# shivangchopra11/MedMoE

Measured on AMD Instinct MI355X. Metric: image-text pairs/sec at global batch 1024, higher is better.
Workload: dtype bf16; 1 GPU; cfg2: ViT-B/16 + 12-layer text tower (frozen), 8 experts top-2, 224x224x3 + 77 tokens, fwd+bwd+clip+Adam; global_batch=1024, per_gpu_batch=1024, parallelism=dp1

## Files before the change

medmoe_amd/csrc/embed.hip:

```cpp
#include "common.h"

template <typename InT>
__global__ __launch_bounds__(256) void patchify_kernel(const InT* __restrict__ img, bf16_t* __restrict__ out, int B,
                                                       int C, int H, int W, int p, int ld) {
  const int gw = W / p, gh = H / p;
  const long long total = (long long)B * C * H * gw;
  for (long long i = blockIdx.x * 256LL + threadIdx.x; i < total; i += (long long)gridDim.x * 256) {
    const int gx = i % gw;
    long long r = i / gw;
    const int y = r % H; r /= H;
    const int c = r % C;
    const int b = r / C;
    const int gy = y / p, py = y - gy * p;
    const InT* src = img + (((long long)b * C + c) * H + y) * W + gx * p;
    bf16_t* dst = out + ((long long)b * gh * gw + gy * gw + gx) * ld + c * p * p + py * p;
    for (int k = 0; k < p; ++k) {
      if constexpr (sizeof(InT) == 4) dst[k] = f2bf(src[k]); else dst[k] = src[k];
    }
  }
}

extern "C" int medmoe_patchify_ld(const void* img, void* out, int B, int C, int H, int W, int patch, int in_f32, int ld,
                                  hipStream_t stream) {
  if (!img || !out) return MM_ERR_ARG;
  if (B <= 0 || C <= 0 || patch <= 0 || (H % patch) || (W % patch) || ld < C * patch * patch || (ld % 8)) return MM_ERR_SHAPE;
  const long long total = (long long)B * C * H * (W / patch);
  const int grid = (int)min((total + 255) / 256, (long long)256 * 16);
  if (in_f32)
    hipLaunchKernelGGL(patchify_kernel<float>, dim3(grid), dim3(256), 0, stream, (const float*)img, (bf16_t*)out, B, C, H, W, patch, ld);
  else
    hipLaunchKernelGGL(patchify_kernel<bf16_t>, dim3(grid), dim3(256), 0, stream, (const bf16_t*)img, (bf16_t*)out, B, C, H, W, patch, ld);
  return mm_check_launch();
}

extern "C" int medmoe_patchify(const void* img, void* out, int B, int C, int H, int W, int patch, int in_f32,
                               hipStream_t stream) {
  if ((C * patch * patch) % 8) return MM_ERR_SHAPE;
  return medmoe_patchify_ld(img, out, B, C, H, W, patch, in_f32, C * patch * patch, stream);
}

__global__ __launch_bounds__(256) void init_tokens_kernel(bf16_t* __restrict__ x, const float* __restrict__ cls,
                                                          const float* __restrict__ pos, int B, int Nt, int D) {
  const long long total = (long long)B * Nt * D / 4;
  for (long long i = blockIdx.x * 256LL + threadIdx.x; i < total; i += (long long)gridDim.x * 256) {
    const long long e = i * 4;
    const int col = e % D;
    const int t = (e / D) % Nt;
    float4 v = *(const float4*)(pos + (long long)t * D + col);
    if (t == 0) {
      const float4 c = *(const float4*)(cls + col);
      v.x += c.x; v.y += c.y; v.z += c.z; v.w += c.w;
    }
    uint2 o; o.x = pack2bf(v.x, v.y); o.y = pack2bf(v.z, v.w);
    *(uint2*)(x + e) = o;
  }
}

extern "C" int medmoe_init_tokens(void* x, const float* cls, const float* pos, int B, int Nt, int D,
                                  hipStream_t stream) {
  if (!x || !cls || !pos) return MM_ERR_ARG;
  if (B <= 0 || Nt <= 0 || D <= 0 || (D % 4)) return MM_ERR_SHAPE;
  const long long total = (long long)B * Nt * D / 4;
  const int grid = (int)min((total + 255) / 256, (long long)256 * 16);
  hipLaunchKernelGGL(init_tokens_kernel, dim3(grid), dim3(256), 0, stream, (bf16_t*)x, cls, pos, B, Nt, D);
  return mm_check_launch();
}

__global__ __launch_bounds__(256) void pos_cls_grad_kernel(const bf16_t* __restrict__ dx, float* __restrict__ dpos,
                                                           float* __restrict__ dcls, int B, int Nt, int D) {
  const int t = blockIdx.x, col = (blockIdx.y * 256 + threadIdx.x) * 2;
  if (col >= D) return;
  const bf16_t* src = dx + (long long)t * D + col;
  const long long bs = (long long)Nt * D;
  float s0 = 0.f, s1 = 0.f;
  int b = 0;
  for (; b + 8 <= B; b += 8) {
    uint32_t v[8];
#pragma unroll
    for (int u = 0; u < 8; ++u) v[u] = *(const uint32_t*)(src + (b + u) * bs);
#pragma unroll
    for (int u = 0; u < 8; ++u) { s0 += __uint_as_float(v[u] << 16); s1 += __uint_as_float(v[u] & 0xffff0000u); }
  }
  for (; b < B; ++b) {
    const uint32_t v = *(const uint32_t*)(src + b * bs);
    s0 += __uint_as_float(v << 16); s1 += __uint_as_float(v & 0xffff0000u);
  }
  dpos[(long long)t * D + col] += s0; dpos[(long long)t * D + col + 1] += s1;
  if (t == 0) { dcls[col] += s0; dcls[col + 1] += s1; }
}

extern "C" int medmoe_pos_cls_grad(const void* dx, float* dpos, float* dcls, int B, int Nt, int D,
                                   hipStream_t stream) {
  if (!dx || !dpos || !dcls) return MM_ERR_ARG;
  if (B <= 0 || Nt <= 0 || D <= 0 || (D % 2)) return MM_ERR_SHAPE;
  hipLaunchKernelGGL(pos_cls_grad_kernel, dim3(Nt, (D + 511) / 512), dim3(256), 0, stream, (const bf16_t*)dx, dpos,
                     dcls, B, Nt, D);
  return mm_check_launch();
}

__global__ __launch_bounds__(256) void text_embed_ln_kernel(const int* __restrict__ ids, const int* __restrict__ tts,
                                                            const float* __restrict__ word, const float* __restrict__ pos,
                                                            const float* __restrict__ type, const float* __restrict__ gamma,
                                                            const float* __restrict__ beta, bf16_t* __restrict__ out,
                                                            int rows, int T, int D, int vocab, float eps, const int* __restrict__ src_of_row,
                                                            const int* __restrict__ rows_dev) {
  const int lane = threadIdx.x & 63, wid = threadIdx.x >> 6;
  const int n4 = D >> 2;
  if (rows_dev) rows = min(rows, *rows_dev);
  for (int row = blockIdx.x * 4 + wid; row < rows; row += gridDim.x * 4) {
    const int src = src_of_row ? src_of_row[row] : row;
    const int t = src % T;
    int id = ids[src]; id = min(max(id, 0), vocab - 1);
    const int tt = tts ? min(max(tts[src], 0), 1) : 0;
    float4 v[8];
    float s = 0.f;
#pragma unroll
    for (int i = 0; i < 8; ++i) {
      const int c = lane + i * 64;
      if (c < n4) {
        const float4 a = *(const float4*)(word + (long long)id * D + c * 4);
        const float4 p = *(const float4*)(pos + (long long)t * D + c * 4);
        const float4 y = *(const float4*)(type + (long long)tt * D + c * 4);
        v[i] = make_float4(a.x + p.x + y.x, a.y + p.y + y.y, a.z + p.z + y.z, a.w + p.w + y.w);
        s += v[i].x + v[i].y + v[i].z + v[i].w;
      }
    }
    const float mean = wave_sum(s) / (float)D;
    float sq = 0.f;
#pragma unroll
    for (int i = 0; i < 8; ++i)
      if (lane + i * 64 < n4) {
        const float a = v[i].x - mean, b = v[i].y - mean, c = v[i].z - mean, d = v[i].w - mean;
        sq += a * a + b * b + c * c + d * d;
      }
    const float rstd = rsqrtf(wave_sum(sq) / (float)D + eps);
#pragma unroll
    for (int i = 0; i < 8; ++i) {
      const int c = lane + i * 64;
      if (c < n4) {
        const float4 g = *(const float4*)(gamma + c * 4), b = *(const float4*)(beta + c * 4);
        uint2 o;
        o.x = pack2bf((v[i].x - mean) * rstd * g.x + b.x, (v[i].y - mean) * rstd * g.y + b.y);
        o.y = pack2bf((v[i].z - mean) * rstd * g.z + b.z, (v[i].w - mean) * rstd * g.w + b.w);
        *(uint2*)(out + (long long)row * D + c * 4) = o;
      }
    }
  }
}

extern "C" int medmoe_text_embed_ln(const int* ids, const int* type_ids, const float* word, const float* pos,
                                    const float* type, const float* gamma, const float* beta, void* out,
                                    int B, int T, int D, int vocab, float eps, hipStream_t stream) {
  if (!ids || !word || !pos || !type || !gamma || !beta || !out) return MM_ERR_ARG;
  if (B <= 0 || T <= 0 || D <= 0 || (D % 4) || D > 2048 || vocab <= 0) return MM_ERR_SHAPE;
  const int rows = B * T;
  const int grid = min((rows + 3) / 4, 256 * 8);
  hipLaunchKernelGGL(text_embed_ln_kernel, dim3(grid), dim3(256), 0, stream, ids, type_ids, word, pos, type, gamma,
                     beta, (bf16_t*)out, rows, T, D, vocab, eps, (const int*)nullptr, (const int*)nullptr);
  return mm_check_launch();
}

__global__ __launch_bounds__(1024) void text_pack_kernel(const unsigned char* __restrict__ mask, int* __restrict__ tok_row,
                                                         int* __restrict__ src_of_row, int* __restrict__ seq_off, int* __restrict__ count,
                                                         int B, int T) {
  __shared__ int sh[1024];
  const int b = threadIdx.x;
  int n = 0;
  if (b < B)
    for (int t = 0; t < T; ++t) n += mask[b * T + t] ? 1 : 0;
  sh[b] = n;
  __syncthreads();
  for (int o = 1; o < 1024; o <<= 1) {
    const int v = (b >= o) ? sh[b - o] : 0;
    __syncthreads();
    sh[b] += v;
    __syncthreads();
  }
  if (b < B) {
    int r = sh[b] - n;
    seq_off[b] = r;
    for (int t = 0; t < T; ++t) {
      if (mask[b * T + t]) { tok_row[b * T + t] = r; src_of_row[r] = b * T + t; ++r; }
      else tok_row[b * T + t] = -1;
    }
    if (b == B - 1) { seq_off[B] = sh[b]; count[0] = sh[b]; }
  }
}

extern "C" int medmoe_text_pack(const unsigned char* mask, int* tok_row, int* src_of_row, int* seq_off, int* count, int B, int T,
                                hipStream_t stream) {
  if (!mask || !tok_row || !src_of_row || !seq_off || !count) return MM_ERR_ARG;
  if (B <= 0 || B > 1024 || T <= 0) return MM_ERR_SHAPE;
  hipLaunchKernelGGL(text_pack_kernel, dim3(1), dim3(1024), 0, stream, mask, tok_row, src_of_row, seq_off, count, B, T);
  return mm_check_launch();
}

__global__ __launch_bounds__(256) void segment_map_kernel(const void* __restrict__ ids_, int ids64, const unsigned char* __restrict__ is_cont,
                                                          const unsigned char* __restrict__ starts_bracket, int* __restrict__ seg,
                                                          int* __restrict__ cap, int B, int T, int vocab, int sep_id) {
  const int b = blockIdx.x * 256 + threadIdx.x;
  if (b >= B) return;
  auto id_at = [&](int t) -> int {
    const long long v = ids64 ? ((const long long*)ids_)[(long long)b * T + t] : (long long)((const int*)ids_)[(long long)b * T + t];
    return (int)min(max(v, 0ll), (long long)vocab - 1);
  };
  int sep_pos = T;
  for (int t = 0; t < T; ++t)
    if (id_at(t) == sep_id) { sep_pos = t; break; }
  int c = -1, at_sep = 0;
  for (int t = 0; t < T; ++t) {
    const int id = id_at(t);
    const bool st = t == 0 || (t <= sep_pos && !is_cont[id]);
    c += st ? 1 : 0;
    seg[(long long)b * T + t] = c;
    if (t == sep_pos) at_sep = c;
  }
  const int n_words = sep_pos < T ? at_sep + 1 : c;
  int prev = -1, n_real = 0;
  for (int t = 0; t < T; ++t) {
    const int w = seg[(long long)b * T + t];
    const bool keep = t <= sep_pos && w < n_words;
    if (keep && w != prev) {
      n_real += starts_bracket[id_at(t)] ? 0 : 1;
      prev = w;
    }
    if (!keep) seg[(long long)b * T + t] = -1;
  }
  cap[b] = n_real + 1;
}

__global__ __launch_bounds__(256) void segment_map_wave_kernel(const void* __restrict__ ids_, int ids64, const unsigned char* __restrict__ is_cont,
                                                               const unsigned char* __restrict__ starts_bracket, int* __restrict__ seg,
                                                               int* __restrict__ cap, int B, int T, int vocab, int sep_id) {
  const int lane = threadIdx.x & 63;
  const int b = blockIdx.x * 4 + (threadIdx.x >> 6);
  if (b >= B) return;
  int id[2], cont[2], brk[2];
#pragma unroll
  for (int u = 0; u < 2; ++u) {
    const int t = 2 * lane + u;
    id[u] = -1; cont[u] = 0; brk[u] = 0;
    if (t < T) {
      const long long v = ids64 ? ((const long long*)ids_)[(long long)b * T + t] : (long long)((const int*)ids_)[(long long)b * T + t];
      id[u] = (int)min(max(v, 0ll), (long long)vocab - 1);
      cont[u] = is_cont[id[u]]; brk[u] = starts_bracket[id[u]];
    }
  }
  int sep_pos = T;
#pragma unroll
  for (int u = 1; u >= 0; --u) if (2 * lane + u < T && id[u] == sep_id) sep_pos = 2 * lane + u;
#pragma unroll
  for (int m = 32; m > 0; m >>= 1) sep_pos = min(sep_pos, __shfl_xor(sep_pos, m, 64));
  int st[2];
#pragma unroll
  for (int u = 0; u < 2; ++u) { const int t = 2 * lane + u; st[u] = (t < T && (t == 0 || (t <= sep_pos && !cont[u]))) ? 1 : 0; }
  int incl = st[0] + st[1];
#pragma unroll
  for (int m = 1; m < 64; m <<= 1) { const int v = __shfl_up(incl, m, 64); if (lane >= m) incl += v; }
  const int base = incl - st[0] - st[1];
  int c[2] = {base + st[0] - 1, base + st[0] + st[1] - 1};
  const int probe = sep_pos < T ? sep_pos : T - 1;
  int at = (probe >> 1) == lane ? c[probe & 1] : 0;
#pragma unroll
  for (int m = 32; m > 0; m >>= 1) at += __shfl_xor(at, m, 64);
  const int n_words = sep_pos < T ? at + 1 : at;
  int n_real = 0;
#pragma unroll
  for (int u = 0; u < 2; ++u) {
// ... 393 lines not shown
```

medmoe_amd/csrc/gemm.hip:

```cpp
#include "common.h"
#include "det_plan.h"
#include <utility>

#define BM 128
#define BN 128
#define BK 64

__device__ __attribute__((aligned(256))) bf16_t g_zero_page[2048];

struct GemmNTArgs {
  const bf16_t* A; const bf16_t* B; void* C;
  const float* bias; const bf16_t* residual; bf16_t* aux;
  const int* a_rowmap; const int* c_rowmap; const int4* tiles; const int* tile_count;
  long long strideB; long long strideBias;
  int M, N, K, lda, ldb, ldc, ldr, ldaux;
  int n_tiles_n, max_tiles_m;
  float alpha; int epi; int out_f32; int col_perm;
  const int* m_dev;
};

static int g_use_nt256 = 1, g_use_nt512 = 1, g_use_tn512 = 1, g_tn_rows = 1024, g_nt_max_grid = 256, g_use_scores512 = 1, g_use_nt4w = 1, g_use_tn4w = 1, g_tn_min_rows = 2048, g_tn_rows4w = 0, g_scores_skip_epi = 0;
#ifdef NT_EXPERIMENT
__device__ int g_nt_dbg_skip = 0;
#define NT_X(...) __VA_ARGS__
#else
#define NT_X(...)
#endif
#ifdef NT_TIMING
__device__ unsigned long long g_nt_timing[8 * 8];
#define NT_T(...) __VA_ARGS__
__device__ __forceinline__ long long nt_clk() {
  __builtin_amdgcn_sched_barrier(0); const long long c = clock64(); __builtin_amdgcn_sched_barrier(0); return c;
}
#else
#define NT_T(...)
#endif
extern int g_attn_resident;
extern int g_sa_rows;
extern int g_attn_rt13;
static int g_last_nt_kernel = -1;
extern "C" int medmoe_last_gemm_nt_kernel() { return g_last_nt_kernel; }
extern int g_ln_one_row;
int g_use_nt_direct = 1;
extern "C" int medmoe_set_option(int key, int value) {
  if (key == 16) { g_ln_one_row = value; return MM_OK; }
  if (key == 17) { g_use_nt_direct = value; return MM_OK; }
  if (key == 1) { g_use_nt256 = value; return MM_OK; }
  if (key == 2) { g_use_nt512 = value; return MM_OK; }
  if (key == 3) { g_use_tn512 = value; return MM_OK; }
  if (key == 4 && value >= 256) { g_tn_rows = value; return MM_OK; }
  if (key == 5 && value >= 1 && value <= 256) { g_nt_max_grid = value; return MM_OK; }
  if (key == 6) { g_use_scores512 = value; return MM_OK; }
  if (key == 7) { g_use_nt4w = value; return MM_OK; }
  if (key == 8) { g_use_tn4w = value; return MM_OK; }
  if (key == 9 && value >= 64) { g_tn_min_rows = value; return MM_OK; }
  if (key == 12) { g_scores_skip_epi = value; return MM_OK; }
  if (key == 15 && (value == 0 || value == 448 || value == 512)) { g_attn_rt13 = value; return MM_OK; }
  if (key == 13 && value >= 0) { g_sa_rows = value; return MM_OK; }
  if (key == 11) { g_attn_resident = value; return MM_OK; }
  if (key == 10 && value >= 0) { g_tn_rows4w = value; return MM_OK; }
  return MM_ERR_ARG;
}

enum { EPI_NONE = 0, EPI_GELU = 1, EPI_RELU = 2, EPI_MUL_DGELU = 3, EPI_MUL_DRELU = 4, EPI_GELU_DAUX = 5, EPI_MUL_AUX = 6 };

struct ParkedTile {
  uint4 c[8];
  int m_base, n_base, n_items, next;
};

typedef unsigned u32x4e_t __attribute__((ext_vector_type(4)));
template <bool PARK, int TM0 = 0, int TMS = 4, int TN0 = 0, int TNS = 4, bool LDSX = false>
__device__ __forceinline__ int nt_epilogue(const GemmNTArgs& p, f32x4_t (&acc)[TMS][TNS], int m_base, int m_end,
                                           int n_base, int group, int frag_row, int frag_q, ParkedTile* park, unsigned lds_x = 0u) {
  int n_stores = 0;
  const int pg = ((frag_q & 1) << 1) | (frag_q >> 1);
  long long mc[4];
  bool mok[4];
#pragma unroll
  for (int tm = 0; tm < 4; ++tm) {
    const int m = m_base + tm * 16 + frag_row;
    mok[tm] = m < m_end;
    const int mr = min(m, m_end - 1);
    mc[tm] = p.c_rowmap ? (long long)p.c_rowmap[mr] : (long long)mr;
  }
  int nn[4];
  bool nok[4];
#pragma unroll
  for (int tn = 0; tn < 4; ++tn) {
    const int n = n_base + tn * 16 + pg * 4;
    nok[tn] = n < p.N;
    nn[tn] = min(n, p.N - 4);
  }
  float4 b4[4];
  if (p.bias) {
    const float* bias = p.bias + (long long)group * p.strideBias;
#pragma unroll
    for (int tn = 0; tn < 4; ++tn) b4[tn] = *(const float4*)(bias + nn[tn]);
  }
  uint2 res[4][4], axv[4][4];
  if (p.residual) {
#pragma unroll
    for (int tm = 0; tm < 4; ++tm)
#pragma unroll
      for (int tn = 0; tn < 4; ++tn) res[tm][tn] = *(const uint2*)(p.residual + mc[tm] * p.ldr + nn[tn]);
  }
  const bool mul_epi = p.epi == EPI_MUL_DGELU || p.epi == EPI_MUL_DRELU || p.epi == EPI_MUL_AUX;
  if (mul_epi) {
#pragma unroll
    for (int tm = 0; tm < 4; ++tm)
#pragma unroll
      for (int tn = 0; tn < 4; ++tn) axv[tm][tn] = *(const uint2*)(p.aux + mc[tm] * p.ldaux + nn[tn]);
  }
  const bool wide = !p.out_f32 && !p.col_perm && (p.N & 7) == 0;
  const bool upper = frag_q >= 2;
  auto store_pair = [&](bf16_t* base, long long ld, int tm, int j, uint2 lo, uint2 hi, bool is_aux) {
    auto r0 = __builtin_amdgcn_permlane32_swap(lo.x, hi.x, false, false);
    auto r1 = __builtin_amdgcn_permlane32_swap(lo.y, hi.y, false, false);
    if constexpr (PARK) {
      if (!is_aux) { park->c[tm * 2 + j] = make_uint4(r0[0], r1[0], r0[1], r1[1]); return; }
    }
    if constexpr (LDSX) {
      const int row_l = (tm & 1) * 16 + frag_row, slot = (2 * j + (upper ? 1 : 0)) * 2 + (frag_q & 1);
      const unsigned a = lds_x + (is_aux ? 4096u : 0u) + row_l * 128 + ((slot ^ ((row_l >> 1) & 7)) << 4);
      const u32x4e_t d = {(unsigned)r0[0], (unsigned)r1[0], (unsigned)r0[1], (unsigned)r1[1]};
      asm volatile("ds_write_b128 %0, %1" :: "v"(a), "v"(d) : "memory");
      return;
    }
// ... 722 lines not shown
    const float f[8] = {lo[i][0], lo[i][1], lo[i][2], lo[i][3], hi[i][0], hi[i][1], hi[i][2], hi[i][3]};
    float o[8], dg[8];
#pragma unroll
    for (int k = 0; k < 4; ++k) {
      if constexpr (GELU) {
        f32x2_t g_, d_;
        gelu_and_grad2((f32x2_t){f[2 * k], f[2 * k + 1]}, g_, d_);
        o[2 * k] = g_[0]; o[2 * k + 1] = g_[1]; dg[2 * k] = d_[0]; dg[2 * k + 1] = d_[1];
      } else {
        const float z0 = __uint_as_float(r[i][k] << 16), z1 = __uint_as_float(r[i][k] & 0xffff0000u);
        o[2 * k] = MUL ? f[2 * k] * z0 : f[2 * k] + z0;
        o[2 * k + 1] = MUL ? f[2 * k + 1] * z1 : f[2 * k + 1] + z1;
      }
    }
    const u32x4e_t pk = {pack2bf(o[0], o[1]), pack2bf(o[2], o[3]), pack2bf(o[4], o[5]), pack2bf(o[6], o[7])};
    __builtin_nontemporal_store(pk, (u32x4e_t*)((bf16_t*)p.C + (long long)(mb + tmh * 16 + i * 8 + rl) * p.ldc + nb + tnq * 16 + c8 * 8));
    if constexpr (GELU) {
      const u32x4e_t pd = {pack2bf(dg[0], dg[1]), pack2bf(dg[2], dg[3]), pack2bf(dg[4], dg[5]), pack2bf(dg[6], dg[7])};
      __builtin_nontemporal_store(pd, (u32x4e_t*)(p.aux + (long long)(mb + tmh * 16 + i * 8 + rl) * p.ldaux + nb + tnq * 16 + c8 * 8));
    }
  }
}
template <int SPEC>
__device__ __forceinline__ int nt4w_epilogue_rows(const GemmNTArgs& p, f32x4_t (&acc)[8][8], int mb, int nb, int frag_row, int frag_q,
                                                  unsigned lx) {
  constexpr bool MUL = (SPEC & 7) == EPI_MUL_AUX;
  asm volatile("" : "+v"(frag_row), "+v"(frag_q));
  const int lane = frag_q * 16 + frag_row, rl = lane >> 3, c8 = lane & 7;
  const int pg = ((frag_q & 1) << 1) | (frag_q >> 1);
  float4 b4[8];
  float zero = 0.f;
  asm volatile("" : "+v"(zero));
#pragma unroll
  for (int tn = 0; tn < 8; ++tn) b4[tn] = (SPEC & 8) ? *(const float4*)(p.bias + nb + tn * 16 + pg * 4) : make_float4(zero, zero, zero, zero);
  u32x4e_t ra[4], rb[4];
  constexpr bool OPERAND = MUL || ((SPEC & 16) != 0);
#define NT4R_LOAD(R, H) do { if constexpr (OPERAND) nt4w_rows_load<MUL>(p, R, H, mb, nb, rl, c8); } while (0)
#define NT4R_HALF(R, H, W) nt4w_rows_half<SPEC, H, W>(p, acc, b4, R, mb, nb, frag_row, pg, rl, c8, lx)
  NT4R_LOAD(ra, 0);
  NT4R_LOAD(rb, 1); NT4R_HALF(ra, 0, 4);
  NT4R_LOAD(ra, 2); NT4R_HALF(rb, 1, 8);
  NT4R_LOAD(rb, 3); NT4R_HALF(ra, 2, 8);
  NT4R_LOAD(ra, 4); NT4R_HALF(rb, 3, 8);
  NT4R_LOAD(rb, 5); NT4R_HALF(ra, 4, 8);
  NT4R_LOAD(ra, 6); NT4R_HALF(rb, 5, 8);
  NT4R_LOAD(rb, 7); NT4R_HALF(ra, 6, 8);
  NT4R_HALF(rb, 7, 4);
#undef NT4R_LOAD
#undef NT4R_HALF
  return ((SPEC & 7) == EPI_GELU_DAUX) ? 64 : 32;
}

template <typename F, int... Is>
__device__ __forceinline__ void static_for_seq(F& f, std::integer_sequence<int, Is...>) { (f(std::integral_constant<int, Is>{}), ...); }
template <int N, typename F>
__device__ __forceinline__ void static_for(F& f) { static_for_seq(f, std::make_integer_sequence<int, N>{}); }
#define DS_READ128(dst, addr, imm) asm volatile("ds_read_b128 %0, %1 offset:%2" : "=v"(dst) : "v"(addr), "n"(imm))
#define STAGE4 (512 * 128)
#ifndef NT4_DSTEP
#define NT4_DSTEP 5
#endif
#ifndef NT4_RS
#define NT4_RS 1
#endif
#define NT4_B1 (16 * NT4_RS + 5)
#ifndef NT4_B2
#define NT4_B2 101
#endif
#ifndef NT4_RS3
#define NT4_RS3 1
#endif
static_assert(NT4_B1 + 2 + 15 * NT4_DSTEP + 2 < NT4_B2, "the DMA pieces must be out before the vmcnt wait");
static_assert(NT4_B2 + 16 * NT4_RS3 < 125, "the last fragment reads need time to land");
__device__ __forceinline__ void wait_vmcnt_4w(int n) {
  if (n == 16) asm volatile("s_waitcnt vmcnt(16)" ::: "memory");
  else if (n >= 63) asm volatile("s_waitcnt vmcnt(63)" ::: "memory");
  else if (n >= 48) asm volatile("s_waitcnt vmcnt(48)" ::: "memory");
  else if (n >= 32) asm volatile("s_waitcnt vmcnt(32)" ::: "memory");
  else if (n >= 24) asm volatile("s_waitcnt vmcnt(24)" ::: "memory");
  else if (n >= 16) asm volatile("s_waitcnt vmcnt(16)" ::: "memory");
  else asm volatile("s_waitcnt vmcnt(0)" ::: "memory");
}

template <int SPEC, bool GROUPED = false>
__global__ __launch_bounds__(256) void gemm_nt4w_kernel(GemmNTArgs p_in) {
  GemmNTArgs p = p_in;
  if (!GROUPED && p.m_dev) { p.M = min(*p.m_dev, p.M); p.max_tiles_m = (p.M + 255) / 256; }
#ifdef NT4_SKIP
  constexpr int dbg4 = NT4_SKIP;
#else
  constexpr int dbg4 = 0;
#endif
  if constexpr (SPEC >= 0) {
    p.epi = SPEC & 7; p.out_f32 = (SPEC >> 6) & 1; p.col_perm = 0; p.alpha = 1.f;
    if (!GROUPED) { p.c_rowmap = nullptr; p.a_rowmap = nullptr; }
    if (!(SPEC & 8)) p.bias = nullptr;
    if (!(SPEC & 16)) p.residual = nullptr;
    if (!(SPEC & 32)) p.aux = nullptr;
    __builtin_assume((p.N & 7) == 0);
    if (SPEC & 8) __builtin_assume(p.bias != nullptr);
    if (SPEC & 16) __builtin_assume(p.residual != nullptr);
    if (SPEC & 32) __builtin_assume(p.aux != nullptr);
  }
#ifdef NT4_NO_XLDS
  constexpr bool XLDS = false;
#else
  constexpr bool XLDS = !GROUPED && SPEC >= 0 && !(SPEC & 64);
#endif
  constexpr bool OPER = XLDS && (((SPEC & 16) != 0 && (SPEC & 7) == EPI_NONE) || (SPEC & 7) == EPI_MUL_AUX || ((SPEC & 7) == EPI_GELU_DAUX && (SPEC & 32) != 0));
  __shared__ __attribute__((aligned(128))) char smem[2 * STAGE4 + (XLDS ? 32768 : 0)];
  const int tid = threadIdx.x, lane = tid & 63, wid = __builtin_amdgcn_readfirstlane(tid >> 6);
  const int wm = wid & 1, wn = wid >> 1;
  const int frag_row = lane & 15, frag_q = lane >> 4;
  const int G = gridDim.x;
  const int my = xcd_remap(blockIdx.x, G);
  const int total = GROUPED ? *p.tile_count * p.n_tiles_n : p.max_tiles_m * p.n_tiles_n;
  const int nk = p.K / 64;
  constexpr int SM = 4, SN = 8;
  struct Tile { int m0, n0, m_end, group; };
  auto decode = [&](int id) -> Tile {
    Tile t;
    if constexpr (GROUPED) {
      const int tm = id / p.n_tiles_n;
      const int4 e = p.tiles[tm];
      t.group = e.x; t.m0 = e.y; t.m_end = e.z; t.n0 = (id - tm * p.n_tiles_n) * 256;
      return t;
    }
    t.group = 0; t.m_end = p.M;
    const int per_super = SM * p.n_tiles_n;
    const int sg = id / per_super, r = id - sg * per_super;
    const int rows = min(SM, p.max_tiles_m - sg * SM);
    const int blk = SN * rows;
    const int nfull = p.n_tiles_n / SN;
    int tile_m, tile_n;
    if (r < nfull * blk) { const int nb = r / blk, w = r - nb * blk; tile_n = nb * SN + (w % SN); tile_m = sg * SM + (w / SN); }
    else {
      const int r2 = r - nfull * blk, nc = p.n_tiles_n - nfull * SN;
      tile_n = nfull * SN + r2 % nc; tile_m = sg * SM + r2 / nc;
    }
    t.m0 = (p.max_tiles_m - 1 - tile_m) * 256; t.n0 = tile_n * 256;
    return t;
  };
  unsigned src[16];
  const char* baseA = (const char*)p.A;
  const char* baseB = (const char*)p.B;
  const unsigned r0 = tid >> 3, c16 = ((tid & 7) ^ (r0 & 7)) * 16;
  auto setup = [&](const Tile& t) {
    const bool gather = GROUPED && p.a_rowmap;
    baseA = (const char*)(p.A + (gather ? 0ll : (long long)t.m0 * p.lda));
    baseB = (const char*)(p.B + (GROUPED ? (long long)t.group * p.strideB : 0ll) + (long long)t.n0 * p.ldb);
    const unsigned limA = t.m_end - 1 - t.m0, limB = p.N - 1 - t.n0;
    const unsigned ldaB = p.lda * 2, ldbB = p.ldb * 2;
    unsigned r0v = r0;
    if constexpr (OPER) asm volatile("" : "+v"(r0v));
#pragma unroll
    for (int i = 0; i < 8; ++i) {
      const unsigned ra = min(i * 32 + r0v, limA);
      if (gather) src[i] = (unsigned)p.a_rowmap[t.m0 + ra] * ldaB + c16;
      else src[i] = __umul24(ra, ldaB) + c16;
      src[8 + i] = __umul24(min(i * 32 + r0v, limB), ldbB) + c16;
    }
  };
  f32x4_t acc[8][8];
  auto zero_acc = [&]() __attribute__((always_inline)) {
#pragma unroll
    for (int i = 0; i < 8; ++i)
#pragma unroll
      for (int j = 0; j < 8; ++j) acc[i][j] = (f32x4_t){0.f, 0.f, 0.f, 0.f};
  };
  const int sig = ((((frag_row >> 2) & 1) << 1 | (frag_row >> 3)) << 2) | (frag_row & 3);
  const unsigned lds0 = (unsigned)(size_t)smem;
  const unsigned offA = lds0 + (wm * 128 + frag_row) * 128 + ((frag_q ^ (frag_row & 7)) << 4);
  const unsigned offB = lds0 + (256 + wn * 128 + sig) * 128 + ((frag_q ^ (sig & 7)) << 4);

  if (my >= total) return;
  const int my_tiles = (total - my + G - 1) / G;
  Tile ct = decode(my);
  setup(ct);
  int lid = my, lk = 0, wb = 0;
  const char* gA = baseA;
  const char* gB = baseB;
  unsigned ldsW = lds0 + wid * 1024;
  auto advance = [&]() __attribute__((always_inline)) {
    wb ^= 1;
    if (++lk == nk) {
      lk = 0; lid += G;
      if (lid < total) { const Tile lt = decode(lid); setup(lt); }
    }
    gA = baseA + lk * 128; gB = baseB + lk * 128;
    ldsW = lds0 + wb * STAGE4 + wid * 1024;
  };
  auto piece = [&](int i) __attribute__((always_inline)) {
    __builtin_amdgcn_global_load_lds(GLB_PTR((i < 8 ? gA : gB) + src[i]), (__attribute__((address_space(3))) void*)(size_t)(ldsW + i * 4096), 16, 0, 0);
  };
  int s_prev = 0;
  NT_T(long long t_wait = 0, t_bar = 0, t_comp = 0, t_epi = 0; const long long t_begin = nt_clk();)
  int rbuf = 0;
  bf16x8_t fa0[8], fb0[8], fa1[8], fb1[8];
  auto iteration = [&](bool last) __attribute__((always_inline)) {
    const unsigned aA1 = (offA + rbuf * STAGE4) ^ 64u, aB1 = (offB + rbuf * STAGE4) ^ 64u;
    const unsigned aA0 = offA + (rbuf ^ 1) * STAGE4, aB0 = offB + (rbuf ^ 1) * STAGE4;
    auto one = [&](auto qc) __attribute__((always_inline)) {
      constexpr int q = decltype(qc)::value, h = q >> 6, tm = (q >> 3) & 7, tn = q & 7;
      if constexpr (h == 0) acc[tm][tn] = __builtin_amdgcn_mfma_f32_16x16x32_bf16(fb0[tn], fa0[tm], acc[tm][tn], 0, 0, 0);
      else acc[tm][tn] = __builtin_amdgcn_mfma_f32_16x16x32_bf16(fb1[tn], fa1[tm], acc[tm][tn], 0, 0, 0);
      if constexpr (q < 16 * NT4_RS && (q % NT4_RS) == NT4_RS - 1) {
        constexpr int g = q / NT4_RS;
        __builtin_amdgcn_sched_barrier(0);
// ... 115 lines not shown
                              int out_f32, int col_perm, hipStream_t stream) {
  return gemm_nt_impl(A, lda, B, ldb, C, ldc, M, N, K, bias, residual, ldr, aux, ldaux, a_rowmap, c_rowmap, tiles, tile_count, max_tiles,
                      strideB, strideBias, alpha, epi, out_f32, col_perm, nullptr, stream);
}

extern "C" int medmoe_gemm_nt_rows(const void* A, int lda, const void* B, int ldb, void* C, int ldc, int M, int N, int K, const float* bias,
                                   const void* residual, int ldr, void* aux, int ldaux, float alpha, int epi, int out_f32, const int* m_dev,
                                   hipStream_t stream) {
  if (!m_dev) return MM_ERR_ARG;
  return gemm_nt_impl(A, lda, B, ldb, C, ldc, M, N, K, bias, residual, ldr, aux, ldaux, nullptr, nullptr, nullptr, nullptr, 0, 0, 0, alpha, epi,
                      out_f32, 0, m_dev, stream);
}

static int gemm_nt_impl(const void* A, int lda, const void* B, int ldb, void* C, int ldc,
                        int M, int N, int K, const float* bias, const void* residual, int ldr,
                        void* aux, int ldaux, const int* a_rowmap, const int* c_rowmap,
                        const int* tiles, const int* tile_count, int max_tiles,
                        long long strideB, long long strideBias, float alpha, int epi,
                        int out_f32, int col_perm, const int* m_dev, hipStream_t stream) {
  if (!A || !B || !C) return MM_ERR_ARG;
  if (M <= 0 || N <= 0 || K <= 0 || (K % 32) != 0 || (N % 4) != 0) return MM_ERR_SHAPE;
  if ((lda % 8) || (ldb % 8) || (ldc % 4) || (residual && (ldr % 4)) || (aux && (ldaux % 4))) return MM_ERR_SHAPE;
  if (epi < 0 || epi > EPI_MUL_AUX) return MM_ERR_ARG;
  if ((epi == EPI_MUL_DGELU || epi == EPI_MUL_DRELU || epi == EPI_MUL_AUX) && !aux) return MM_ERR_ARG;
  if (tiles && (!tile_count || max_tiles <= 0)) return MM_ERR_ARG;
  GemmNTArgs p;
  p.A = (const bf16_t*)A; p.B = (const bf16_t*)B; p.C = C;
  p.bias = bias; p.residual = (const bf16_t*)residual; p.aux = (bf16_t*)aux;
  p.a_rowmap = a_rowmap; p.c_rowmap = c_rowmap; p.tiles = (const int4*)tiles; p.tile_count = tile_count;
  p.strideB = strideB; p.strideBias = strideBias;
  p.M = M; p.N = N; p.K = K; p.lda = lda; p.ldb = ldb; p.ldc = ldc; p.ldr = ldr; p.ldaux = ldaux;
  p.n_tiles_n = (N + BN - 1) / BN;
  p.alpha = alpha; p.epi = epi; p.out_f32 = out_f32; p.col_perm = col_perm; p.m_dev = m_dev;
  const bool fits32 = (long long)M * lda * 2 < (1ll << 32) && (long long)N * ldb * 2 < (1ll << 32);
  const bool plain = !tiles && !a_rowmap && !c_rowmap && !col_perm && M >= 4 * BM2 && g_use_nt256 && (K % BK) == 0;
  const bool big = plain && K >= 3 * BK && fits32;
  const bool tile32 = 256ll * lda * 2 < (1ll << 32) && 256ll * ldb * 2 < (1ll << 32);
  const bool pitch24 = 2ll * lda < (1ll << 24) && 2ll * ldb < (1ll << 24);
  const long long t512 = (long long)((M + 255) / 256) * ((N + 255) / 256), t256 = (long long)((M + 255) / 256) * ((N + 127) / 128);
  const double fill512 = (double)t512 / (double)(((t512 + 255) / 256) * 256), fill256 = (double)t256 / (double)(((t256 + 255) / 256) * 256);
  if (plain && tile32 && g_use_nt512 && K >= 128 && N >= 512 && (!big || fill512 * 1.35 >= fill256)) {
    p.max_tiles_m = (M + 255) / 256;
    p.n_tiles_n = (N + 255) / 256;
    const int grid = min(p.max_tiles_m * p.n_tiles_n, g_nt_max_grid);
    int spec = -1;
    if ((N & 7) == 0 && alpha == 1.f && epi != EPI_RELU && epi != EPI_MUL_DRELU) spec = NT_SPEC(epi, bias ? 1 : 0, residual ? 1 : 0, aux ? 1 : 0) | (out_f32 ? 64 : 0);
    if (g_use_nt4w && spec >= 0 && pitch24) {
      bool done = true;
      switch (spec) {
#define NT_CASE(s) case s: hipLaunchKernelGGL(gemm_nt4w_kernel<s>, dim3(grid), dim3(256), 0, stream, p); break;
        NT_CASE(NT_SPEC(EPI_NONE, 0, 0, 0))
        NT_CASE(NT_SPEC(EPI_NONE, 1, 0, 0))
        NT_CASE(NT_SPEC(EPI_NONE, 1, 1, 0))
        NT_CASE(NT_SPEC(EPI_NONE, 0, 1, 0))
        NT_CASE(NT_SPEC(EPI_GELU, 1, 0, 1))
        NT_CASE(NT_SPEC(EPI_GELU, 1, 0, 0))
        NT_CASE(NT_SPEC(EPI_MUL_DGELU, 0, 0, 1))
        NT_CASE(NT_SPEC(EPI_GELU_DAUX, 1, 0, 1))
        NT_CASE(NT_SPEC(EPI_MUL_AUX, 0, 0, 1))
        NT_CASE(NT_SPEC(EPI_NONE, 0, 0, 0) | 64)
#undef NT_CASE
        default: done = false; break;
      }
      if (done) { g_last_nt_kernel = 4; return mm_check_launch(); }
    }
    g_last_nt_kernel = 2;
    switch (spec) {
#define NT_CASE(s) case s: hipLaunchKernelGGL((gemm_nt512_kernel<s, false>), dim3(grid), dim3(512), 0, stream, p); break;
      NT_CASE(NT_SPEC(EPI_NONE, 0, 0, 0))
      NT_CASE(NT_SPEC(EPI_NONE, 1, 0, 0))
      NT_CASE(NT_SPEC(EPI_NONE, 1, 1, 0))
      NT_CASE(NT_SPEC(EPI_NONE, 0, 1, 0))
      NT_CASE(NT_SPEC(EPI_GELU, 1, 0, 1))
      NT_CASE(NT_SPEC(EPI_GELU, 1, 0, 0))
      NT_CASE(NT_SPEC(EPI_MUL_DGELU, 0, 0, 1))
      NT_CASE(NT_SPEC(EPI_GELU_DAUX, 1, 0, 1))
      NT_CASE(NT_SPEC(EPI_MUL_AUX, 0, 0, 1))
      NT_CASE(NT_SPEC(EPI_NONE, 0, 0, 0) | 64)
#undef NT_CASE
      default: hipLaunchKernelGGL((gemm_nt512_kernel<-1, false>), dim3(grid), dim3(512), 0, stream, p); break;
    }
    return mm_check_launch();
  }
  if (big) {
    g_last_nt_kernel = 1;
    p.max_tiles_m = (M + BM2 - 1) / BM2;
    const int grid = min(p.max_tiles_m * p.n_tiles_n, 256);
    int spec = -1;
    if ((N & 7) == 0 && alpha == 1.f && epi != EPI_RELU && epi != EPI_MUL_DRELU) spec = NT_SPEC(epi, bias ? 1 : 0, residual ? 1 : 0, aux ? 1 : 0) | (out_f32 ? 64 : 0);
    switch (spec) {
#define NT_CASE(s) case s: hipLaunchKernelGGL(gemm_nt256_kernel<s>, dim3(grid), dim3(512), 0, stream, p); break;
      NT_CASE(NT_SPEC(EPI_NONE, 0, 0, 0))
      NT_CASE(NT_SPEC(EPI_NONE, 1, 0, 0))
      NT_CASE(NT_SPEC(EPI_NONE, 1, 1, 0))
      NT_CASE(NT_SPEC(EPI_NONE, 0, 1, 0))
      NT_CASE(NT_SPEC(EPI_GELU, 1, 0, 1))
      NT_CASE(NT_SPEC(EPI_GELU, 1, 0, 0))
      NT_CASE(NT_SPEC(EPI_MUL_DGELU, 0, 0, 1))
      NT_CASE(NT_SPEC(EPI_GELU_DAUX, 1, 0, 1))
      NT_CASE(NT_SPEC(EPI_MUL_AUX, 0, 0, 1))
#undef NT_CASE
      default: hipLaunchKernelGGL(gemm_nt256_kernel<-1>, dim3(grid), dim3(512), 0, stream, p); break;
    }
    return mm_check_launch();
  }
  if (g_use_nt_direct && !tiles && !a_rowmap && !c_rowmap && !col_perm && !m_dev && (K & 63) == 32 && K <= 288 && M >= 4096) {
    const long long waves = (long long)((M + 63) / 64) * ((N + 63) / 64);
    const dim3 dgrid((unsigned)((waves + 3) / 4));
    g_last_nt_kernel = 6;
    int spec = -1;
    if ((N & 7) == 0 && alpha == 1.f && !out_f32 && epi != EPI_RELU && epi != EPI_MUL_DRELU) spec = NT_SPEC(epi, bias ? 1 : 0, residual ? 1 : 0, aux ? 1 : 0);
    switch (spec) {
#define NT_CASE(s) case s: hipLaunchKernelGGL(gemm_nt_direct_kernel<s>, dgrid, dim3(256), 0, stream, p); break;
      NT_CASE(NT_SPEC(EPI_NONE, 0, 0, 0))
      NT_CASE(NT_SPEC(EPI_NONE, 1, 0, 0))
      NT_CASE(NT_SPEC(EPI_NONE, 1, 1, 0))
      NT_CASE(NT_SPEC(EPI_GELU_DAUX, 1, 0, 1))
      NT_CASE(NT_SPEC(EPI_MUL_AUX, 0, 0, 1))
#undef NT_CASE
      default: hipLaunchKernelGGL(gemm_nt_direct_kernel<-1>, dgrid, dim3(256), 0, stream, p); break;
    }
    return mm_check_launch();
  }
  p.max_tiles_m = tiles ? max_tiles : (M + BM - 1) / BM;
  const int grid = min(p.max_tiles_m * p.n_tiles_n, 2 * 256);
  g_last_nt_kernel = 0;
  hipLaunchKernelGGL(gemm_nt_kernel, dim3(grid), dim3(256), 0, stream, p);
  return mm_check_launch();
}

struct GemmTNArgs {
  const bf16_t* G; const bf16_t* X; float* dW; float* db;
  const int* x_rowmap; const int* g_rowmap; const int* row_off;
  long long strideW; long long strideDb;
  int M, Nn, Kk, ldg, ldx, ldw;
  int tiles_n, tiles_k, nsplit, n_groups;
  long long gcol_stride, xcol_stride;
  long long g_chunk_stride; int g_chunk_w;
  const float* gscale; long long gscale_gstride; int gscale_ld;
  float* partial;
  float* db_partial = nullptr;
};

template <bool MAPPED>
__global__ __launch_bounds__(256) void gemm_tn_kernel(GemmTNArgs p) {
  __shared__ __attribute__((aligned(16))) char smem[2 * 32768];
  const int tid = threadIdx.x, lane = tid & 63, wid = tid >> 6;
  const int wn = wid >> 1, wk = wid & 1;
  int id = xcd_remap(blockIdx.x, gridDim.x);
  const int tile_k = id % p.tiles_k; id /= p.tiles_k;
  const int tile_n = id % p.tiles_n; id /= p.tiles_n;
  const int split = id % p.nsplit;
  const int group = id / p.nsplit;
  int r0 = 0, r1 = p.M;
  if (p.row_off) { r0 = p.row_off[group]; r1 = p.row_off[group + 1]; }
  const int chunk = (((r1 - r0 + p.nsplit - 1) / p.nsplit) + BK - 1) / BK * BK;
  const int ms = r0 + split * chunk;
  const int me = min(r1, ms + chunk);
  if (ms >= me) return;
  const int n0 = tile_n * 128, k0 = tile_k * 128;

  const int srow = wid * 4 + (lane >> 4);
  const int schunk = lane & 15;
  const int lds_off = srow * 256 + ((schunk ^ ((srow & 3) << 2)) << 4);
  const bool g_col_ok = (n0 + schunk * 8) < p.Nn;
  const bool x_col_ok = (k0 + schunk * 8) < p.Kk;
// ... 1349 lines not shown
```

medmoe_amd/csrc/moe.hip:

```cpp
#include "common.h"

__global__ __launch_bounds__(256) void mean_tokens_kernel(const bf16_t* __restrict__ x, float* __restrict__ out, int Nt,
                                                          int D, int t0, int cnt) {
#pragma clang fp contract(off)
  const int b = blockIdx.x, col = blockIdx.y * 512 + threadIdx.x * 2;
  if (col >= D) return;
  float a0 = 0.f, a1 = 0.f;
  for (int t = t0; t < t0 + cnt; ++t) {
    const uint32_t v = *(const uint32_t*)(x + ((long long)b * Nt + t) * D + col);
    a0 = a0 + __uint_as_float(v << 16);
    a1 = a1 + __uint_as_float(v & 0xffff0000u);
  }
  out[(long long)b * D + col] = a0 / (float)cnt;
  out[(long long)b * D + col + 1] = a1 / (float)cnt;
}

extern "C" int medmoe_mean_tokens(const void* x, float* out, int B, int Nt, int D, int t0, int cnt,
                                  hipStream_t stream) {
  if (!x || !out) return MM_ERR_ARG;
  if (B <= 0 || D <= 0 || (D % 2) || t0 < 0 || cnt <= 0 || t0 + cnt > Nt) return MM_ERR_SHAPE;
  hipLaunchKernelGGL(mean_tokens_kernel, dim3(B, (D + 511) / 512), dim3(256), 0, stream, (const bf16_t*)x, out, Nt, D, t0, cnt);
  return mm_check_launch();
}

// ... 159 lines not shown
                     ce_scale, dlogits, dh, loss_acc, B, Hd, E, k, parts);
  mm_launch_det_sum(parts, B, 2, loss_acc, stream);
  return mm_check_launch();
}

__global__ __launch_bounds__(256) void router_eval_kernel(const float* __restrict__ probs, const int* __restrict__ labels,
                                                          float* __restrict__ loss_acc, int B, int E) {
  __shared__ float sl[256];
  __shared__ int sh[256];
  const int j = threadIdx.x;
  float loss = 0.f;
  int hits = 0;
  for (int b = j; b < B; b += 256) {
    const float* p = probs + (long long)b * E;
    float m = p[0];
    int am = 0;
    for (int e = 1; e < E; ++e) { m = fmaxf(m, p[e]); if (p[e] > p[am]) am = e; }
    float s = 0.f;
    for (int e = 0; e < E; ++e) s += __expf(p[e] - m);
    const int lab = labels[b];
    if (lab >= 0 && lab < E) loss += -__logf(__expf(p[lab] - m) / s) / (float)B;
    hits += am == lab;
  }
  sl[j] = loss; sh[j] = hits;
  __syncthreads();
  for (int o = 128; o > 0; o >>= 1) {
    if (j < o) { sl[j] += sl[j + o]; sh[j] += sh[j + o]; }
    __syncthreads();
  }
  if (j == 0) {
    float acc = 0.f;
    for (int n = 0; n < sh[0]; ++n) acc += 1.f / (float)B;
    loss_acc[0] = sl[0];
    loss_acc[1] = acc;
  }
}

extern "C" int medmoe_router_eval(const float* probs, const int* labels, float* loss_acc, int B, int E, hipStream_t stream) {
  if (!probs || !labels || !loss_acc) return MM_ERR_ARG;
  if (B <= 0 || E <= 0 || E > ROUTER_MAX_E) return MM_ERR_SHAPE;
  hipLaunchKernelGGL(router_eval_kernel, dim3(1), dim3(256), 0, stream, probs, labels, loss_acc, B, E);
  return mm_check_launch();
}

__global__ __launch_bounds__(256) void sgemm_kernel(const float* __restrict__ A, const float* __restrict__ Bm,
                                                    float* __restrict__ C, int M, int N, int K, long long sam,
                                                    long long sak, long long sbk, long long sbn, long long ldc,
                                                    float alpha, float beta) {
  __shared__ float sA[16][65], sB[16][65];
  const int tx = threadIdx.x & 15, ty = threadIdx.x >> 4;
  const int m0 = blockIdx.y * 64, n0 = blockIdx.x * 64;
  float acc[4][4] = {};
  for (int k0 = 0; k0 < K; k0 += 16) {
    for (int i = threadIdx.x; i < 64 * 16; i += 256) {
      const int kk = i & 15, r = i >> 4;
      sA[kk][r] = (m0 + r < M && k0 + kk < K) ? A[(long long)(m0 + r) * sam + (long long)(k0 + kk) * sak] : 0.f;
      sB[kk][r] = (n0 + r < N && k0 + kk < K) ? Bm[(long long)(k0 + kk) * sbk + (long long)(n0 + r) * sbn] : 0.f;
    }
    __syncthreads();
#pragma unroll
    for (int kk = 0; kk < 16; ++kk) {
      float a[4], b[4];
#pragma unroll
      for (int i = 0; i < 4; ++i) { a[i] = sA[kk][ty * 4 + i]; b[i] = sB[kk][tx * 4 + i]; }
#pragma unroll
      for (int i = 0; i < 4; ++i)
#pragma unroll
        for (int jn = 0; jn < 4; ++jn) acc[i][jn] += a[i] * b[jn];
    }
    __syncthreads();
  }
#pragma unroll
  for (int i = 0; i < 4; ++i)
#pragma unroll
    for (int jn = 0; jn < 4; ++jn) {
      const int m = m0 + ty * 4 + i, n = n0 + tx * 4 + jn;
      if (m < M && n < N) {
        float* c = C + (long long)m * ldc + n;
        *c = alpha * acc[i][jn] + (beta != 0.f ? beta * (*c) : 0.f);
      }
    }
}

extern "C" int medmoe_sgemm(const float* A, const float* Bm, float* C, int M, int N, int K, long long sam,
                            long long sak, long long sbk, long long sbn, long long ldc, float alpha, float beta,
                            hipStream_t stream) {
  if (!A || !Bm || !C) return MM_ERR_ARG;
  if (M <= 0 || N <= 0 || K <= 0) return MM_ERR_SHAPE;
  hipLaunchKernelGGL(sgemm_kernel, dim3((N + 63) / 64, (M + 63) / 64), dim3(256), 0, stream, A, Bm, C, M, N, K, sam,
                     sak, sbk, sbn, ldc, alpha, beta);
  return mm_check_launch();
}

__global__ __launch_bounds__(256) void dispatch_kernel(const int* __restrict__ idx, int n_items, int E, int P,
                                                       int* __restrict__ slot_of, int* __restrict__ item_of_slot,
                                                       int* __restrict__ expert_of_slot, int* __restrict__ row_off,
                                                       int* __restrict__ tiles, int* __restrict__ tile_count,
                                                       int max_tiles) {
  __shared__ unsigned short cnt[256][ROUTER_MAX_E];
  __shared__ int off[ROUTER_MAX_E + 1], t128[ROUTER_MAX_E + 1], t256[ROUTER_MAX_E + 1];
  const int tid = threadIdx.x;
  const int per = (n_items + 255) / 256;
  const int lo = min(tid * per, n_items), hi = min(lo + per, n_items);
  for (int e = 0; e < E; ++e) cnt[tid][e] = 0;
  for (int i = lo; i < hi; ++i) cnt[tid][idx[i]] += 1;
  __syncthreads();
  if (tid < E) {
    int run = 0;
    for (int t = 0; t < 256; ++t) { const int c = cnt[t][tid]; cnt[t][tid] = (unsigned short)run; run += c; }
    t128[tid + 1] = run;
  }
  __syncthreads();
  if (tid == 0) {
    off[0] = 0;
    for (int e = 0; e < E; ++e) off[e + 1] = off[e] + t128[e + 1];
    t128[0] = 0; t256[0] = 0;
    for (int e = 0; e < E; ++e) {
      const int rows = (off[e + 1] - off[e]) * P;
      t128[e + 1] = t128[e] + (rows + 127) / 128;
      t256[e + 1] = t256[e] + (rows + 255) / 256;
    }
    tile_count[0] = min(t128[E], max_tiles);
    tile_count[1] = min(t256[E], max_tiles);
  }
  __syncthreads();
  if (tid <= E) row_off[tid] = off[tid] * P;
  for (int i = lo; i < hi; ++i) {
    const int e = idx[i];
    const int s = off[e] + cnt[tid][e]++;
    slot_of[i] = s; item_of_slot[s] = i; expert_of_slot[s] = e;
  }
  int* tiles2 = tiles + max_tiles * 4;
  for (int e = 0; e < E; ++e) {
    const int r0 = off[e] * P, r1 = off[e + 1] * P;
    for (int t = tid; t128[e] + t < min(t128[e + 1], max_tiles); t += 256) {
      int* q = tiles + (t128[e] + t) * 4;
      q[0] = e; q[1] = r0 + t * 128; q[2] = r1; q[3] = 0;
    }
    for (int t = tid; t256[e] + t < min(t256[e + 1], max_tiles); t += 256) {
      int* q = tiles2 + (t256[e] + t) * 4;
      q[0] = e; q[1] = r0 + t * 256; q[2] = r1; q[3] = 0;
    }
  }
}

__global__ __launch_bounds__(256) void rowmap_kernel(const int* __restrict__ item_of_slot, int k, int P, int Nt,
                                                     int R, int* __restrict__ rowmap) {
  for (int r = blockIdx.x * 256 + threadIdx.x; r < R; r += gridDim.x * 256) {
    const int s = r / P, p = r - s * P;
    rowmap[r] = (item_of_slot[s] / k) * Nt + 1 + p;
  }
}

extern "C" int medmoe_dispatch(const int* idx, int B, int k, int E, int P, int Nt, int* slot_of, int* item_of_slot,
                               int* expert_of_slot, int* row_off, int* tiles, int* tile_count, int max_tiles,
                               int* rowmap, hipStream_t stream) {
  if (!idx || !slot_of || !item_of_slot || !expert_of_slot || !row_off || !tiles || !tile_count || !rowmap) return MM_ERR_ARG;
  if (B <= 0 || k < 1 || E < 1 || E > ROUTER_MAX_E || P <= 0 || Nt < P + 1 || (long long)B * k >= 65536) return MM_ERR_SHAPE;
  const int R = B * k * P;
  if (max_tiles < (R + 127) / 128 + E) return MM_ERR_SHAPE;
  hipLaunchKernelGGL(dispatch_kernel, dim3(1), dim3(256), 0, stream, idx, B * k, E, P, slot_of, item_of_slot,
                     expert_of_slot, row_off, tiles, tile_count, max_tiles);
  hipLaunchKernelGGL(rowmap_kernel, dim3(min((R + 255) / 256, 2048)), dim3(256), 0, stream, item_of_slot, k, P, Nt, R, rowmap);
  return mm_check_launch();
}

#define SA_S 4
template <int DCH, int HCH>
__global__ __launch_bounds__(256) void scale_attn_fwd_kernel(const bf16_t* __restrict__ G, const bf16_t* __restrict__ H1,
                                                             const float* __restrict__ w2, const float* __restrict__ b2,
                                                             const int* __restrict__ expert_of_slot, int P,
                                                             bf16_t* __restrict__ out, float* __restrict__ wts, int R,
                                                             int Do, int Dh) {
// ... 486 lines not shown
```

Baseline: 4881 pairs/s.

## Add MFMA fp32 sgemm, vectorized patchify, wave-parallel text pack, grouped 256-row GEMM path

```diff
diff --git a/medmoe_amd/csrc/embed.hip b/medmoe_amd/csrc/embed.hip
--- a/medmoe_amd/csrc/embed.hip
+++ b/medmoe_amd/csrc/embed.hip
@@ -20,10 +20,32 @@
   }
 }
 
+__global__ __launch_bounds__(256) void patchify_vec_kernel(const bf16_t* __restrict__ img, bf16_t* __restrict__ out, int B, int C, int H, int W,
+                                                           int p, int ld) {
+  const int w8 = W >> 3, p8 = p >> 3, gw = W / p, gh = H / p;
+  const long long total = (long long)B * C * H * w8;
+  for (long long i = blockIdx.x * 256LL + threadIdx.x; i < total; i += (long long)gridDim.x * 256) {
+    const int x8 = i % w8;
+    long long r = i / w8;
+    const int y = r % H; r /= H;
+    const int c = r % C;
+    const int b = r / C;
+    const int gx = x8 / p8, pc = x8 - gx * p8;
+    const int gy = y / p, py = y - gy * p;
+    *(uint4*)(out + ((long long)b * gh * gw + gy * gw + gx) * ld + c * p * p + py * p + pc * 8) = *(const uint4*)(img + i * 8);
+  }
+}
+
 extern "C" int medmoe_patchify_ld(const void* img, void* out, int B, int C, int H, int W, int patch, int in_f32, int ld,
                                   hipStream_t stream) {
   if (!img || !out) return MM_ERR_ARG;
   if (B <= 0 || C <= 0 || patch <= 0 || (H % patch) || (W % patch) || ld < C * patch * patch || (ld % 8)) return MM_ERR_SHAPE;
+  if (!in_f32 && patch % 8 == 0 && ((uintptr_t)img | (uintptr_t)out) % 16 == 0) {
+    const long long pieces = (long long)B * C * H * (W / 8);
+    hipLaunchKernelGGL(patchify_vec_kernel, dim3((int)min((pieces + 255) / 256, (long long)256 * 16)), dim3(256), 0, stream, (const bf16_t*)img,
+                       (bf16_t*)out, B, C, H, W, patch, ld);
+    return mm_check_launch();
+  }
   const long long total = (long long)B * C * H * (W / patch);
   const int grid = (int)min((total + 255) / 256, (long long)256 * 16);
   if (in_f32)
@@ -164,26 +186,38 @@
                                                          int* __restrict__ src_of_row, int* __restrict__ seq_off, int* __restrict__ count,
                                                          int B, int T) {
   __shared__ int sh[1024];
-  const int b = threadIdx.x;
-  int n = 0;
-  if (b < B)
-    for (int t = 0; t < T; ++t) n += mask[b * T + t] ? 1 : 0;
-  sh[b] = n;
+  const int b = threadIdx.x, lane = threadIdx.x & 63, wid = threadIdx.x >> 6;
+  for (int c = wid; c < 1024; c += 16) {
+    int n = 0;
+    if (c < B)
+      for (int t0 = 0; t0 < T; t0 += 64) {
+        const int t = t0 + lane;
+        n += __popcll(__ballot(t < T && mask[c * T + t]));
+      }
+    if (lane == 0) sh[c] = n;
+  }
   __syncthreads();
+  const int n = sh[b];
   for (int o = 1; o < 1024; o <<= 1) {
     const int v = (b >= o) ? sh[b - o] : 0;
     __syncthreads();
     sh[b] += v;
     __syncthreads();
   }
-  if (b < B) {
-    int r = sh[b] - n;
-    seq_off[b] = r;
-    for (int t = 0; t < T; ++t) {
-      if (mask[b * T + t]) { tok_row[b * T + t] = r; src_of_row[r] = b * T + t; ++r; }
-      else tok_row[b * T + t] = -1;
-    }
-    if (b == B - 1) { seq_off[B] = sh[b]; count[0] = sh[b]; }
+  if (b < B) seq_off[b] = sh[b] - n;
+  if (b == B - 1) { seq_off[B] = sh[b]; count[0] = sh[b]; }
+  for (int c = wid; c < B; c += 16) {
+    int r = c ? sh[c - 1] : 0;
+    for (int t0 = 0; t0 < T; t0 += 64) {
+      const int t = t0 + lane;
+      const bool on = t < T && mask[c * T + t];
+      const unsigned long long m = __ballot(on);
+      if (on) {
+        const int row = r + __popcll(m & ((1ull << lane) - 1));
+        tok_row[c * T + t] = row; src_of_row[row] = c * T + t;
+      } else if (t < T) tok_row[c * T + t] = -1;
+      r += __popcll(m);
+    }
   }
 }
 
diff --git a/medmoe_amd/csrc/gemm.hip b/medmoe_amd/csrc/gemm.hip
--- a/medmoe_amd/csrc/gemm.hip
+++ b/medmoe_amd/csrc/gemm.hip
@@ -41,9 +41,11 @@
 static int g_last_nt_kernel = -1;
 extern "C" int medmoe_last_gemm_nt_kernel() { return g_last_nt_kernel; }
 extern int g_ln_one_row;
+extern int g_sgemm_plain;
 int g_use_nt_direct = 1;
 extern "C" int medmoe_set_option(int key, int value) {
   if (key == 16) { g_ln_one_row = value; return MM_OK; }
+  if (key == 18) { g_sgemm_plain = value; return MM_OK; }
   if (key == 17) { g_use_nt_direct = value; return MM_OK; }
   if (key == 1) { g_use_nt256 = value; return MM_OK; }
   if (key == 2) { g_use_nt512 = value; return MM_OK; }
@@ -932,8 +934,9 @@
   else asm volatile("s_waitcnt vmcnt(0)" ::: "memory");
 }
 
-template <int SPEC, bool GROUPED = false>
+template <int SPEC, bool GROUPED = false, bool ROWS256 = false>
 __global__ __launch_bounds__(256) void gemm_nt4w_kernel(GemmNTArgs p_in) {
+  static_assert(GROUPED || !ROWS256, "ROWS256 is a GROUPED build");
   GemmNTArgs p = p_in;
   if (!GROUPED && p.m_dev) { p.M = min(*p.m_dev, p.M); p.max_tiles_m = (p.M + 255) / 256; }
 #ifdef NT4_SKIP
@@ -964,7 +967,7 @@
   const int frag_row = lane & 15, frag_q = lane >> 4;
   const int G = gridDim.x;
   const int my = xcd_remap(blockIdx.x, G);
-  const int total = GROUPED ? *p.tile_count * p.n_tiles_n : p.max_tiles_m * p.n_tiles_n;
+  const int total = GROUPED && !ROWS256 ? *p.tile_count * p.n_tiles_n : p.max_tiles_m * p.n_tiles_n;
   const int nk = p.K / 64;
   constexpr int SM = 4, SN = 8;
   struct Tile { int m0, n0, m_end, group; };
@@ -972,8 +975,10 @@
     Tile t;
     if constexpr (GROUPED) {
       const int tm = id / p.n_tiles_n;
+      t.n0 = (id - tm * p.n_tiles_n) * 256;
+      if constexpr (ROWS256) { t.group = 0; t.m0 = tm * 256; t.m_end = min(t.m0 + 256, p.M); return t; }
       const int4 e = p.tiles[tm];
-      t.group = e.x; t.m0 = e.y; t.m_end = e.z; t.n0 = (id - tm * p.n_tiles_n) * 256;
+      t.group = e.x; t.m0 = e.y; t.m_end = e.z;
       return t;
     }
     t.group = 0; t.m_end = p.M;
@@ -1255,6 +1260,14 @@
     }
     return mm_check_launch();
   }
+  if (g_use_nt4w && c_rowmap && !tiles && !a_rowmap && !col_perm && !m_dev && !out_f32 && alpha == 1.f && epi == EPI_NONE && bias && residual &&
+      !aux && K >= 128 && (K % BK) == 0 && (N & 7) == 0 && (ldc & 7) == 0 && (ldr & 7) == 0 && tile32 && pitch24) {
+    p.max_tiles_m = (M + 255) / 256;
+    p.n_tiles_n = (N + 255) / 256;
+    g_last_nt_kernel = 5;
+    hipLaunchKernelGGL((gemm_nt4w_kernel<NT_SPEC(EPI_NONE, 1, 1, 0), true, true>), dim3(min(p.max_tiles_m * p.n_tiles_n, 256)), dim3(256), 0, stream, p);
+    return mm_check_launch();
+  }
   if (big) {
     g_last_nt_kernel = 1;
     p.max_tiles_m = (M + BM2 - 1) / BM2;
diff --git a/medmoe_amd/csrc/moe.hip b/medmoe_amd/csrc/moe.hip
--- a/medmoe_amd/csrc/moe.hip
+++ b/medmoe_amd/csrc/moe.hip
@@ -265,13 +265,85 @@
     }
 }
 
+typedef float sg_f32x16 __attribute__((ext_vector_type(16)));
+constexpr int SG_BK = 32;
+template <bool KFAST>
+__device__ __forceinline__ void sg_coord(int tid, int i, int& kk, int& r) {
+  if constexpr (KFAST) { kk = tid & 31; r = (tid >> 5) + 8 * i; } else { r = tid & 63; kk = (tid >> 6) + 4 * i; }
+}
+template <bool KA, bool KB>
+__global__ __launch_bounds__(256) void sgemm_mfma_kernel(const float* __restrict__ A, const float* __restrict__ Bm, float* __restrict__ C,
+                                                         int M, int N, int K, long long sam, long long sak, long long sbk, long long sbn,
+                                                         long long ldc, float alpha, float beta) {
+  __shared__ float sA[SG_BK][65], sB[SG_BK][65];
+  const int tid = threadIdx.x, lane = tid & 63, wid = tid >> 6;
+  const int m0 = blockIdx.y * 64, n0 = blockIdx.x * 64;
+  const int wm = (wid >> 1) * 32, wn = (wid & 1) * 32;
+  const int fc = lane & 31, fh = lane >> 5;
+  float ra[8], rb[8];
+  auto fetch = [&](int k0) {
+#pragma unroll
+    for (int i = 0; i < 8; ++i) {
+      int kk, r;
+      sg_coord<KA>(tid, i, kk, r);
+      ra[i] = (m0 + r < M && k0 + kk < K) ? A[(long long)(m0 + r) * sam + (long long)(k0 + kk) * sak] : 0.f;
+      sg_coord<KB>(tid, i, kk, r);
+      rb[i] = (n0 + r < N && k0 + kk < K) ? Bm[(long long)(k0 + kk) * sbk + (long long)(n0 + r) * sbn] : 0.f;
+    }
+  };
+  auto park = [&]() {
+#pragma unroll
+    for (int i = 0; i < 8; ++i) {
+      int kk, r;
+      sg_coord<KA>(tid, i, kk, r);
+      sA[kk][r] = ra[i];
+      sg_coord<KB>(tid, i, kk, r);
+      sB[kk][r] = rb[i];
+    }
+  };
+  sg_f32x16 acc;
+#pragma unroll
+  for (int j = 0; j < 16; ++j) acc[j] = 0.f;
+  fetch(0);
+  park();
+  __syncthreads();
+  for (int k0 = 0; k0 < K; k0 += SG_BK) {
+    const bool more = k0 + SG_BK < K;
+    if (more) fetch(k0 + SG_BK);
+#pragma unroll
+    for (int ks = 0; ks < SG_BK; ks += 2)
+      acc = __builtin_amdgcn_mfma_f32_32x32x2f32(sA[ks + fh][wm + fc], sB[ks + fh][wn + fc], acc, 0, 0, 0);
+    __syncthreads();
+    if (more) {
+      park();
+      __syncthreads();
+    }
+  }
+  const int n = n0 + wn + fc;
+#pragma unroll
+  for (int j = 0; j < 16; ++j) {
+    const int m = m0 + wm + (j & 3) + 8 * (j >> 2) + 4 * fh;
+    if (m < M && n < N) {
+      float* c = C + (long long)m * ldc + n;
+      *c = alpha * acc[j] + (beta != 0.f ? beta * (*c) : 0.f);
+    }
+  }
+}
+
+int g_sgemm_plain = 0;
 extern "C" int medmoe_sgemm(const float* A, const float* Bm, float* C, int M, int N, int K, long long sam,
                             long long sak, long long sbk, long long sbn, long long ldc, float alpha, float beta,
                             hipStream_t stream) {
   if (!A || !Bm || !C) return MM_ERR_ARG;
   if (M <= 0 || N <= 0 || K <= 0) return MM_ERR_SHAPE;
-  hipLaunchKernelGGL(sgemm_kernel, dim3((N + 63) / 64, (M + 63) / 64), dim3(256), 0, stream, A, Bm, C, M, N, K, sam,
-                     sak, sbk, sbn, ldc, alpha, beta);
+  const dim3 grid((N + 63) / 64, (M + 63) / 64);
+#define SGEMM_LAUNCH(KERNEL) hipLaunchKernelGGL(KERNEL, grid, dim3(256), 0, stream, A, Bm, C, M, N, K, sam, sak, sbk, sbn, ldc, alpha, beta)
+  if (M == 1 || g_sgemm_plain) SGEMM_LAUNCH(sgemm_kernel);
+  else if (sak == 1 && sbk == 1) SGEMM_LAUNCH((sgemm_mfma_kernel<true, true>));
+  else if (sak == 1) SGEMM_LAUNCH((sgemm_mfma_kernel<true, false>));
+  else if (sbk == 1) SGEMM_LAUNCH((sgemm_mfma_kernel<false, true>));
+  else SGEMM_LAUNCH((sgemm_mfma_kernel<false, false>));
+#undef SGEMM_LAUNCH
   return mm_check_launch();
 }
 
```

Measured after the change: 4906 pairs/s, median of 6. About the same (+0.5%).
